# timdestan/go-raytracer

Measured on AMD Instinct MI355X. Metric: Mrays/s (primary+shadow+reflect) at 4K depth=6; 1/2/4/8-GPU scaling, higher is better.
Workload: dtype f64; 1 GPU; c3: cylinder + cube + sphere (cone substitute) over a reflective plane, 4 lights, 3840x2160, depth 6; width=3840, height=2160, depth=6, lights=4, objects=4, parallelism=rows1-interleaved, frames_in_flight=2, schedule=auto, kernel=specialised, accel=bvh+cull

## Files before the change

### go-raytracer_amd/csrc/rt_kernel.hip

```cpp
#pragma clang fp contract(off)

#include <hip/hip_runtime.h>

#include <dlfcn.h>
#include <errno.h>
#include <fcntl.h>
#include <hip/hiprtc.h>
#include <sys/syscall.h>
#include <sys/wait.h>
#include <unistd.h>

#include <algorithm>
#include <atomic>
#include <chrono>
#include <condition_variable>
#include <cstdlib>
#include <functional>
#include <thread>
#include <cmath>
#include <array>
#include <cstdio>
#include <utility>
#include <cstring>
#include <limits>
// ... 398 lines not shown

int align16(int v) { return (v + 15) & ~15; }

}

struct SpecKey {
  int lds = 1, bvh = 0, csg = 0, nobj = 0;
  std::string kinds;
  int kmask = 0, feat = 0, nlights = 0;
  int pow_bits = 7;
  int nocull = 0;
  int quads = 0;
  int share = 0;
  int far = 1;
  std::string str() const {
    return std::to_string(lds) + ":" + std::to_string(bvh) + ":" + std::to_string(csg) + ":" + std::to_string(nobj) + ":" + kinds + ":" +
           std::to_string(kmask) + ":" + std::to_string(feat) + ":" + std::to_string(nlights) + ":" + std::to_string(pow_bits) +
           ":" + std::to_string(nocull) + ":" + std::to_string(quads) + ":" + std::to_string(share) + ":" + std::to_string(far);
  }
};

struct LaunchPlan {
  const void* fn = nullptr;
  int shmem_fixed = -1, frames = 0, per_cu = 0, lds_levels = 0, lds_full = 0;
};

struct rt_context {
  int device = 0;
  int last_waves = 0, launches = 0;
  int sched = RT_SCHED_AUTO;
  int inflight = 1;
  LaunchPlan plan;
  unsigned long long* wdiag = nullptr;
  int cus = 0;
  int lds_per_cu = 0, lds_per_block = 0;
  int grid_lds = 0, grid_glb = 0;
  DevScene sc;
  bool has_scene = false;
  uint64_t* jump = nullptr;
  unsigned int* queue = nullptr;
  int qset = 0;
  unsigned long long* stats = nullptr;
  unsigned long long* stats_part = nullptr;
  int stats_parts = 0;
  double* stack = nullptr;
  double* vm_global = nullptr;
  size_t vm_global_bytes = 0;
// ... 1583 lines not shown
  const bool use_stream = !lds && !s.use_bvh && !s.has_csg && (spec_extra || !(spec && !(c->accel & RT_ACCEL_CULL)));
  const bool quads = sch == SCH_QUADS || (sch == SCH_PAIRS && !spec);
  const void* kfn = k_kernels[kernel_index(lds, s.use_bvh, s.has_csg, quads, s.ext_code)];
  const bool share = spec && share_m == RT_SHARE_GROUP;
  const int stream_off = board_off + (share ? BOARD_BYTES : 0);
  const int frames_off = stream_off + (use_stream ? WAVES_PER_WG * SCH * (GEO * (int)sizeof(double) + (int)sizeof(int)) : 0);
  int shmem = frames_off;
  auto occupancy = [&](int bytes) {
    int n = 0;
    if (spec) {
      if (hipModuleOccupancyMaxActiveBlocksPerMultiprocessor(&n, spec, WG, bytes) != hipSuccess) n = 0;
    } else if (hipOccupancyMaxActiveBlocksPerMultiprocessor(&n, kfn, WG, bytes) != hipSuccess) {
      n = 0;
    }
    return n;
  };
  const void* plan_fn = spec ? (const void*)spec : kfn;
  const int frames = std::max(1, s.depth - 1);
  LaunchPlan& pl = c->plan;
  const bool plan_hit = pl.fn == plan_fn && pl.shmem_fixed == shmem && pl.frames == frames;
  int per_cu = plan_hit ? pl.per_cu : occupancy(shmem);
  if (per_cu <= 0) per_cu = 1;
  const int level_bytes = WAVES_PER_WG * CORE * 64 * (int)sizeof(double);
  const int ext_bytes = WAVES_PER_WG * EXT_ROWS * 64 * (int)sizeof(double);
  int lds_levels = plan_hit ? pl.lds_levels : 0, lds_full = plan_hit ? pl.lds_full : 0;
  if (!plan_hit && c->lds_per_cu > 0 && c->lds_per_block > 0) {
    const int avail = std::min(c->lds_per_block, c->lds_per_cu / std::min(per_cu, 8)) - shmem;
    if (const char* e = rt_getenv("RT_LDS_FULL")) lds_full = std::max(0, std::min(frames, atoi(e)));
    while (lds_full > 0 && lds_full * (ext_bytes + level_bytes) > avail) lds_full--;
    lds_levels = std::max(lds_full, std::min(frames, (avail - lds_full * ext_bytes) / level_bytes));
    if (const char* e = rt_getenv("RT_LDS_LEVELS")) lds_levels = std::max(lds_full, std::min(lds_levels, atoi(e)));
    while (lds_levels > 0 && occupancy(shmem + lds_levels * level_bytes + lds_full * ext_bytes) < per_cu) {
      lds_levels--;
      lds_full = std::min(lds_full, lds_levels);
    }
  }
  if (!plan_hit) pl = LaunchPlan{plan_fn, shmem, frames, per_cu, lds_levels, lds_full};
  const int ext_off = shmem + lds_levels * level_bytes;
  shmem = ext_off + lds_full * ext_bytes;
  static const bool dbg = rt_getenv("RT_DEBUG_LAUNCH") != nullptr;
  if (dbg)
    fprintf(stderr, "[launch] blocks/CU %d, LDS/block %d B (fixed %d, frame cores %d levels, full frames %d levels), frames %d\n",
            per_cu, shmem, frames_off, lds_levels, lds_full, frames);
  const int grid = c->cus * std::min(per_cu, 8);
  c->last_waves = grid * WAVES_PER_WG;
  c->launches++;
  if (grid * WAVES_PER_WG > c->stack_waves) return fail(RT_E_INVALID, "frame stack smaller than the grid");
  if (spec && share_m == RT_SHARE_DEVICE) {
    const size_t need = (size_t)c->stack_waves * 64 * frames;
    if (need != c->gslots || frames != c->gframes) {
      (void)hipFree(c->gboard);
      c->gboard = nullptr;
      c->gslots = 0;
      if (hipExtMallocWithFlags((void**)&c->gboard, need * GS_REC * sizeof(uint64_t), hipDeviceMallocUncached) !=
          hipSuccess)
        return fail(RT_E_NOMEM, "device-wide work-sharing slots");
      if (!c->gring && hipExtMallocWithFlags((void**)&c->gring, (size_t)GS_RING * sizeof(uint64_t),
                                             hipDeviceMallocUncached) != hipSuccess)
        return fail(RT_E_NOMEM, "device-wide work-sharing ring");
      if (!c->gctl && hipExtMallocWithFlags((void**)&c->gctl, GS_CTL_U64 * sizeof(uint64_t), hipDeviceMallocUncached) !=
                          hipSuccess)
        return fail(RT_E_NOMEM, "device-wide work-sharing control");
      HIP_TRY(hipMemsetAsync(c->gboard, 0, need * GS_REC * sizeof(uint64_t), st));
      HIP_TRY(hipMemsetAsync(c->gring, 0, (size_t)GS_RING * sizeof(uint64_t), st));
      HIP_TRY(hipMemsetAsync(c->gctl, 0, GS_CTL_U64 * sizeof(uint64_t), st));
      c->gslots = need;
      c->gframes = frames;
    }
  }
  Params P;
  std::memset(&P, 0, sizeof P);
  P.lds_frames_off = frames_off;
  P.lds_levels = lds_levels;
  P.lds_full = lds_full;
  P.stream_off = stream_off;
  P.lds_ext_off = ext_off;
  P.qmask_off = qmask_off;
  P.jump_off = jump_off;
  P.board_off = board_off;
  P.gboard = c->gboard;
  P.gring = c->gring;
  P.gctl = c->gctl;
  P.gslots = c->gslots;
  P.gset = c->qset;
  P.off_geo = s.off_geo;
  P.off_shade = s.off_shade;
  P.off_mats = s.off_mats;
  P.off_lights = s.off_lights;
  P.off_kind = s.off_kind;
  P.off_objmat = s.off_objmat;
  P.off_pref = s.off_prefb;
  P.off_csg = s.off_csg;
  P.off_code = s.off_code;
  P.off_consts = s.off_consts;
  P.off_entry = s.off_entry;
  P.lds_vm_off = vm_off;
  P.vm_global = c->vm_global;
  P.blob_bytes = s.blob_bytes;
  P.jump = c->jump;
// ... 346 lines not shown
```

### go-raytracer_amd/csrc/rt_render.h

```cpp
#pragma once
#pragma clang fp contract(off)

#ifndef __HIPCC_RTC__
#include <hip/hip_runtime.h>
#endif

#include "rt_abi.h"
#include "rt_device.h"

#ifndef RT_CULL
#define RT_CULL 1
#endif
#ifndef RT_SHARE
#define RT_SHARE 0
#endif
#ifndef RT_PAIRS
#define RT_PAIRS 0
#endif
#ifndef RT_FAR_SHIFT
#define RT_FAR_SHIFT 1
#endif
#ifndef RT_GS_POLL
#define RT_GS_POLL 3
#endif
// ... 48 lines not shown
enum { SCH = 32 };
enum { SHADOW_CHECK = 8 };
enum { ST_SHADOW = 0, ST_TRACED = 1, ST_SHADED = 2, ST_SURFERR = 3, ST_STESTS = 4, ST_COUNT = ST_STESTS + RT_NUM_KINDS,
       ST_PHASE = 16, N_PHASE = 10, ST_BVHDIAG = 26, ST_EXDIAG = 34, ST_SHDIAG = 48, ST_PASSDIAG = 54,
       ST_CLOCKSTEP = 60, ST_LANEDIAG = 61 ,
       ST_WATCHDOG = 63,
       STATS_PART = 16  };
enum { SH_POST_S = 0, SH_POST_T = 1, SH_CLAIM = 2, SH_RECLAIM = 3, SH_WAIT = 4, SH_SPIN = 5 };
#ifdef RT_PHASE_TIMING
#define SHDIAG(k) atomicAdd(P.stats + ST_SHDIAG + (k), 1ull)
#else
#define SHDIAG(k) (void)0
#endif
enum { S_IDLE = 0, S_TRACE = 1, S_SHADE = 2, S_DONE = 3 };
enum { LDS_MAX_BYTES = 40 * 1024 };
enum { JUMP_ENTRIES = 20 * 4 };

__device__ __forceinline__ int est_x(int pts, unsigned int k) { return pts == 1 ? TILE / 2 : 2 + 4 * (int)(k & 1u); }
__device__ __forceinline__ int est_y(int pts, unsigned int k) { return pts == 1 ? TILE / 2 : 2 + 4 * (int)((k >> 1) & 1u); }

struct Params {
  int lds_frames_off;
  int lds_levels;
  int lds_full;
  int lds_ext_off;
  int stream_off;
  int qmask_off;
  int jump_off;
  int off_geo, off_shade, off_mats, off_lights, off_kind, off_objmat, off_pref, off_csg, off_code, off_consts,
      off_entry, blob_bytes;
  int lds_vm_off;
  double* vm_global;
  const uint64_t* jump;
  unsigned int* queue;
  unsigned int* queue_next;
  unsigned long long* stats;
  unsigned long long* stats_part;
  unsigned long long* wdiag;
  double* stack;
  uint32_t* out;
  int width, height, depth, nobj, nlights, y0, y1, tiles_x;
  int trow0, trow_stride;
  unsigned int total_slots;
  int frames;
  const float* bvh_nodes;
  const double* bvh_geo;
  const int* planes;
  int nplanes, bvh_stack_off;
// ... 34 lines not shown
            m[8] * d.x + m[9] * d.y + m[10] * d.z);
}
template <typename MP>
__device__ __forceinline__ Ray to_obj(MP m, const Ray& r) {
  Ray l;
  l.o = to_obj_o(m, r.o);
  l.d = to_obj_d(m, r.d);
  return l;
}
__device__ __forceinline__ bool ax_mag(double x, bool zero_ok) {
  const uint32_t e = ((uint32_t)__double2hiint(x) >> 20) & 0x7ffu;
  return e - 123u < 1800u || (zero_ok && x == 0.0);
}
__device__ __forceinline__ bool axis_o_ok(d3 o) { return ax_mag(o.x, true) && ax_mag(o.y, true) && ax_mag(o.z, true); }
__device__ __forceinline__ bool axis_d_ok(d3 d) { return ax_mag(d.x, false) && ax_mag(d.y, false) && ax_mag(d.z, false); }
__device__ __forceinline__ d3 axis_o(const double* a, d3 o) {
  return mk(a[0] * o.x + a[1], a[2] * o.y + a[3], a[4] * o.z + a[5]);
}
__device__ __forceinline__ d3 axis_d(const double* a, d3 d) { return mk(a[0] * d.x, a[2] * d.y, a[4] * d.z); }

typedef const __attribute__((address_space(4))) double* cdptr;
typedef const __attribute__((address_space(4))) float* cfptr;
typedef const __attribute__((address_space(4))) int* ciptr;
__device__ __forceinline__ const float* as_f(const double* p) { return reinterpret_cast<const float*>(p); }
__device__ __forceinline__ cfptr as_f(cdptr p) { return (cfptr)p; }
__device__ __forceinline__ const int* as_i(const double* p) { return reinterpret_cast<const int*>(p); }
__device__ __forceinline__ ciptr as_i(cdptr p) { return (ciptr)p; }
template <int N>
struct RecN {
  double m[N];
};
typedef RecN<12> Rec12;
typedef RecN<6> Rec6;
typedef RecN<3> Rec3;
enum { AXIS_REC = 8, UNI_REC = 4 };
template <int N, typename PT>
__device__ __forceinline__ RecN<N> ld_rec(PT p) {
  RecN<N> r;
#pragma unroll
  for (int q = 0; q < N; q++) r.m[q] = p[q];
  return r;
}
struct LeafRec {
  RecN<12> R;
  float cx, cy, cz, cr;
  int i, k;
// ... 820 lines not shown
    uint64_t t_ = stamp();                \
    asm volatile("; @phase_end " #k ::: "memory"); \
    ph_acc[k] += t_ - ph_t0_;             \
    ph_t0_ = t_;                          \
  } while (0)
#else
#define PH_BEGIN() (void)0
#define PH_MARK(k) (void)0
#endif

#ifdef RT_EXACT_DIAG
#define EXDIAG(k, sh, b)                                                                    \
  do {                                                                                      \
    const uint64_t act_ = wave_ballot(1), m_ = wave_ballot(b);                                    \
    if ((int)(threadIdx.x & 63) == __ffsll((long long)act_) - 1) {                          \
      atomicAdd(P.stats + ST_EXDIAG + 2 * (k) + (sh), (unsigned long long)__popcll(m_));    \
      atomicAdd(P.stats + ST_EXDIAG + 2 * RT_NUM_KINDS + (sh), 1ull);                       \
    }                                                                                       \
  } while (0)
#else
#define EXDIAG(k, sh, b) (void)0
#endif

__device__ __forceinline__ double* frame_ptr(double* base, int frame) { return base + (size_t)frame * FRAME_FIELDS * 64; }
__device__ __forceinline__ void st3(double* f, int field, d3 v) {
  f[(field + 0) * 64] = v.x;
  f[(field + 1) * 64] = v.y;
  f[(field + 2) * 64] = v.z;
}
__device__ __forceinline__ d3 ld3(const double* f, int field) {
  return mk(f[(field + 0) * 64], f[(field + 1) * 64], f[(field + 2) * 64]);
}

__device__ __forceinline__ int core_gfield(int c) { return c < 3 ? c : (c == 3 ? 9 : 10); }

enum { FL_TMODE = 1, FL_HASR = 2, FL_HAST = 4, FL_STAGE = 8, FL_VMMAT = 16, FL_FORKED = 32, FL_TASK = 64 };
enum { PK_SLOT = 8, PK_MAT = 32 };
#define PK_SLOT_OF(packed) ((int)(((packed) >> PK_SLOT) & 0xffffff))

enum { SHARE_SPINS = 1 << 16,
       SHARE_SLEEP = 127,
       SHARE_SAMPLES = 1 };
enum { NSLOT = 64, SLOTS_PER_WAVE = NSLOT / WAVES_PER_WG, S_WAIT = 4, S_RESUME = 5 };
enum { S_ADV = 6 };
struct Board {
  unsigned long long post;
  unsigned long long done;
  unsigned int wfree[WAVES_PER_WG];
  int nidle;
  int nactive;
  int pad[2];
  double ray[NSLOT][6];
  int meta[NSLOT][2];
  uint32_t lw[WG];
};
__device__ __forceinline__ int lw_own_end(uint32_t w) { return (int)(w & 7u); }
__device__ __forceinline__ int lw_task(uint32_t w) { return (int)((w >> 3) & 127u) - 1; }
// ... 286 lines not shown
  S.mats = reinterpret_cast<const double*>(base + P.off_mats);
  const double* G = reinterpret_cast<const double*>(base + P.off_lights);
  S.lights = G + GLOB;
  S.kind = reinterpret_cast<const int*>(base + P.off_kind);
  S.objmat = reinterpret_cast<const int*>(base + P.off_objmat);
  S.pref = reinterpret_cast<const uint32_t*>(base + P.off_pref);
  S.csg = reinterpret_cast<const int*>(base + P.off_csg);
  S.code = reinterpret_cast<const uint32_t*>(base + P.off_code);
  S.entry = reinterpret_cast<const int*>(base + P.off_entry);
  S.consts = reinterpret_cast<const uint64_t*>(base + P.off_consts);
#ifdef RT_SPEC_NOBJ
  const cdptr sgeo = (cdptr)(blob + P.off_geo);
#endif
  const cdptr cs_geo = (cdptr)(blob + P.off_geo);
  const ciptr cs_kind = (ciptr)(blob + P.off_kind);
  const ciptr cs_csg = (ciptr)(blob + P.off_csg);
#define CSG_ARGS cs_geo, cs_kind, cs_csg
#define CSG_G(i, g) (cs_geo + (size_t)(i) * GEO)
#define LTP(li) (S.lights + (size_t)(li) * LGT)
#define SHP(i) (S.shade + (size_t)(i) * SHD)

  const int lane = (int)(threadIdx.x & 63);
  const int wslot = (int)(blockIdx.x * WAVES_PER_WG + (threadIdx.x >> 6));
  double* stk = P.stack + (size_t)wslot * ((size_t)P.frames * FRAME_FIELDS * 64) + lane;
  const int lds_lv = P.lds_levels;
  double* lfr = reinterpret_cast<double*>(smem + P.lds_frames_off) +
                (size_t)(threadIdx.x >> 6) * (lds_lv * CORE * 64) + lane;
  auto core_ld = [&](int level, int c) -> double {
    if (level < lds_lv) return lfr[(level * CORE + c) * 64];
    return frame_ptr(stk, level)[core_gfield(c) * 64];
  };
  const int lds_full = P.lds_full;
  double* lext = reinterpret_cast<double*>(smem + P.lds_ext_off) + (size_t)(threadIdx.x >> 6) * (lds_full * EXT_ROWS * 64) + lane;
  auto ext = [&](int level) -> double* {
    return level < lds_full ? lext + (size_t)level * EXT_ROWS * 64 : frame_ptr(stk, level) + FR_EXT * 64;
  };
  auto core_st = [&](int level, int c, double v) {
    if (level < lds_lv)
      lfr[(level * CORE + c) * 64] = v;
    else
      frame_ptr(stk, level)[core_gfield(c) * 64] = v;
  };
  double* vmrec;
  if constexpr (LDS)
    vmrec = reinterpret_cast<double*>(smem + P.lds_vm_off) + (size_t)threadIdx.x * MAT;
  else
    vmrec = P.vm_global + ((size_t)wslot * 64 + lane) * MAT;
  constexpr bool STREAM = !LDS && !BVH && !CSG;
  double* sbuf = reinterpret_cast<double*>(smem + P.stream_off) + (size_t)(threadIdx.x >> 6) * (SCH * GEO);
  int* skind = reinterpret_cast<int*>(smem + P.stream_off + WAVES_PER_WG * SCH * GEO * (int)sizeof(double)) +
               (threadIdx.x >> 6) * SCH;
  auto stream_objects = [&](auto&& body) {
    constexpr int PER = SCH * GEO * (int)sizeof(double) / 16 / 64;
    const uint4* src = reinterpret_cast<const uint4*>(S.geo);
    uint4* dst = reinterpret_cast<uint4*>(sbuf);
    const int lane_ = (int)(threadIdx.x & 63);
    uint4 pre[PER];
    int pk = 0;
    auto fetch = [&](int c0) {
      const int n16 = min(SCH, P.nobj - c0) * (GEO * (int)sizeof(double) / 16);
#pragma unroll
      for (int q = 0; q < PER; q++) {
        const int idx = lane_ + q * 64;
        pre[q] = idx < n16 ? src[(size_t)c0 * (GEO * sizeof(double) / 16) + idx] : make_uint4(0, 0, 0, 0);
// ... 89 lines not shown
  uint32_t lane_cost = 0;
#endif
#endif

  const double W1 = (double)(P.width - 1), H1 = (double)(P.height - 1);

  auto gen_ray = [&]() {
    double dx = pcg_float64(rng) - 0.5;
    double dy = pcg_float64(rng) - 0.5;
    const double vw = G[9], vh = G[10];
    double u = ((double)px + dx) / W1 * vw - vw / 2.0;
    double v = ((double)py + dy) / H1 * vh - vh / 2.0;
    ray.o = mk(u, -v, 0.0);
    ray.d = norm(sub(ray.o, eye));
  };

  auto sample_rng = [&](int x, int y, int k) {
    const int ry = y % 20;
    const uint64_t* j = P.jump + (ry * 4 + k) * 4;
    return pcg_jump(Pcg{0xDEADULL ^ (uint64_t)x, 0xBEEFULL ^ (uint64_t)(y - ry)}, j[0], j[1], j[2], j[3]);
  };
  auto wait_slot = [&]() -> int {
    if (RT_SHARE == 1 && !QD && sp == 0) return lw_fork(Bd->lw[threadIdx.x], sample);
    return PK_SLOT_OF(__double_as_longlong(core_ld(sp - 1, 4)));
  };
  auto advance_sample = [&](uint32_t w) {
    for (;;) {
      if (P.est_out && sample == 1) {
        state = S_IDLE;
        return;
      }
      if (PR && sample == ((lane & 1) ? 4 : 2)) {
        state = S_DONE;
        return;
      }
      if (sample == 4) {
        d3 c = scale(sum, 1.0 / 4.0);
        uint32_t r8 = go_f64_to_u32(c.x * 65535.0) >> 8;
        uint32_t g8 = go_f64_to_u32(c.y * 65535.0) >> 8;
        uint32_t b8 = go_f64_to_u32(c.z * 65535.0) >> 8;
#ifdef RT_COST_MAP
        P.out[pout] = lane_cost;
        lane_cost = 0;
#else
        const uint32_t v = (r8 & 0xffu) | ((g8 & 0xffu) << 8) | ((b8 & 0xffu) << 16) | 0xff000000u;
        held_px = pout;
        held_val = v;
// ... 23 lines not shown
      }
      sum = add(sum, board_take(Bd, q));
      sample++;
    }
  };

  auto unwind = [&](bool have_res, d3 res, bool pf_valid, long long pf_packed, d3 pf_lw, double pf_kr) {
    while (wave_any(have_res)) {
      if (have_res) {
        if (sp == 0) {
          if constexpr (QD) {
            sum = res;
            state = S_DONE;
          } else {
            if (PR && (lane & 1))
              (sample == 2 ? sum : sum2) = res;
            else
              sum = add(sum, res);
            sample++;
            state = S_ADV;
          }
          have_res = false;
        } else {
          double* f = frame_ptr(stk, sp - 1);
          long long packed;
          if (pf_valid)
            packed = pf_packed;
          else
            packed = __double_as_longlong(core_ld(sp - 1, 4));
          int fl = (int)(packed & 0xff);
          if (RT_SHARE && __builtin_expect((fl & FL_TASK) != 0, 0)) {
            if constexpr (RT_SHARE == 2)
              gs_deliver(P.gboard, PK_SLOT_OF(packed), res);
            else
              board_deliver(Bd, PK_SLOT_OF(packed), res);
            sp = 0;
            state = S_IDLE;
            have_res = false;
          } else if ((fl & FL_HASR) && (fl & FL_HAST) && !(fl & FL_STAGE)) {
            double* e = ext(sp - 1);
            const d3 first = res;
            bool here = true;
            core_st(sp - 1, 4, __longlong_as_double(packed | FL_STAGE));
            if (RT_SHARE && __builtin_expect((fl & FL_FORKED) != 0, 0)) {
              const int q = PK_SLOT_OF(packed);
              if (RT_SHARE == 2 ? gs_reclaim(P.gboard, q) : board_reclaim(Bd, q)) {
                SHDIAG(SH_RECLAIM);
                if (RT_SHARE == 1) board_free(Bd, q);
              } else if (RT_SHARE == 2 ? gs_done(P.gboard, q) : board_done(Bd, q)) {
                here = false;
                res = RT_SHARE == 2 ? gs_take(P.gboard, q) : board_take(Bd, q);
              } else {
                SHDIAG(SH_WAIT);
                here = false;
                state = S_WAIT;
                have_res = false;
              }
            }
            if (here) {
              ray.o = ld3(e, 0);
              ray.d = ld3(e, 3);
              state = S_TRACE;
              have_res = false;
            }
            st3(e, 0, first);
          } else {
            const double* FM = S.mats + (size_t)(packed >> PK_MAT) * MAT;
            d3 R = mk(0, 0, 0), Tr = mk(0, 0, 0);
            if ((fl & FL_HASR) && (fl & FL_HAST)) {
              R = ld3(ext(sp - 1), 0);
              Tr = res;
            } else if (fl & FL_HASR) {
              R = res;
            } else {
              Tr = res;
            }
            d3 lw;
            double kr;
            if (pf_valid) {
              lw = pf_lw;
              kr = pf_kr;
            } else {
              lw = mk(core_ld(sp - 1, 0), core_ld(sp - 1, 1), core_ld(sp - 1, 2));
              kr = core_ld(sp - 1, 3);
            }
            d3 fcol;
            double frefl;
            if (spec_feat(SF_VM) && (fl & FL_VMMAT)) {
              fcol = ld3(f, FR_COL);
              frefl = f[FR_REFL * 64];
            } else {
              fcol = mk(FM[0], FM[1], FM[2]);
              frefl = FM[3];
            }
            res = combine((fl & FL_TMODE) != 0, lw, fcol, frefl, kr, R, Tr);
            sp--;
          }
          pf_valid = false;
        }
      }
    }
  };

  PH_BEGIN();
#ifdef RT_PHASE_TIMING
  const uint64_t life_t0 = ph_t0_;
  uint64_t last_grab = life_t0, nchunk_taken = 0;
#endif
  uint32_t guard_iters = 0;
  for (;;) {
    if (++guard_iters > (1u << 26)) {
      if (lane == 0) atomicAdd(P.stats + ST_WATCHDOG, 1ull);
      break;
// ... 170 lines not shown
        if (lane == 0) {
          gt = gs_ld(g_tail);
          if (!gs_helper || (guard_iters & 7u) == 0u || gt != gs_t) {
            nid = (int)gs_ld32(g_nidle);
            gh = gs_ld(g_head);
          } else {
            nid = gs_nid;
            gh = gs_h;
          }
        }
        gs_nid = __builtin_amdgcn_readfirstlane(nid);
        gs_h = rfl64(gh);
        gs_t = rfl64(gt);
      }
      const int nid = gs_nid;
      const uint64_t gh = gs_h, gt = gs_t;
      const long long outstanding = (long long)(gt - gh);
      const int want = nid - (int)min(outstanding, (long long)(1 << 30));
      if (__builtin_expect(want > 0 && outstanding < GS_RSH / 2, 0)) {
        const bool busy_lane = state == S_TRACE || state == S_SHADE || state == S_WAIT;
        int L = -1;
        if (busy_lane)
          for (int l = min(sp - 1, P.depth - 1 - GS_MIN_LEVELS); l >= 0; l--) {
            const int f = (int)(__double_as_longlong(core_ld(l, 4)) & 0xff);
            if (f & FL_TASK) break;
            if ((f & (FL_HASR | FL_HAST | FL_STAGE | FL_FORKED)) == (FL_HASR | FL_HAST)) L = l;
          }
        const uint64_t cm = wave_ballot(L >= 0);
        if (cm) {
          const int npost = min((int)__popcll(cm), want);
          const int rk = (int)__builtin_amdgcn_mbcnt_hi((unsigned int)(cm >> 32),
                                                        __builtin_amdgcn_mbcnt_lo((unsigned int)cm, 0u));
          const bool post = L >= 0 && rk < npost;
          int q = 0;
          if (post) {
            SHDIAG(SH_POST_T);
            q = (wslot * 64 + lane) * P.frames + L;
            uint64_t* r = gs_slot(P.gboard, q);
            const double* e = ext(L);
            const d3 o = ld3(e, 0), dd = ld3(e, 3);
            gs_st(r + 0, (uint64_t)__double_as_longlong(o.x));
            gs_st(r + 1, (uint64_t)__double_as_longlong(o.y));
            gs_st(r + 2, (uint64_t)__double_as_longlong(o.z));
            gs_st(r + 3, (uint64_t)__double_as_longlong(dd.x));
            gs_st(r + 4, (uint64_t)__double_as_longlong(dd.y));
            gs_st(r + 5, (uint64_t)__double_as_longlong(dd.z));
            gs_st(r + 6, (uint64_t)(L + 1));
            gs_drain();
            gs_st(r + 7, GS_POSTED);
            const long long pk = __double_as_longlong(core_ld(L, 4));
            core_st(L, 4, __longlong_as_double(pk | FL_FORKED | ((long long)q << PK_SLOT)));
          }
          gs_drain();
          uint64_t t0 = 0;
          if (lane == 0) t0 = __hip_atomic_fetch_add(g_tail, (uint64_t)npost, __ATOMIC_RELAXED, RT_AG_SCOPE);
          t0 = rfl64(t0);
          if (post) {
            const uint64_t t = t0 + (uint64_t)rk;
            gs_st(g_ring + (t & (GS_RSH - 1)), (t << 32) | (uint32_t)q);
          }
        }
      }
      uint64_t il = exhausted ? wave_ballot(state == S_IDLE) : 0ull;
      int cshard = gshard;
      uint64_t ch = gh;
      bool ctry = outstanding > 0;
      if (GS_SH > 1 && il != 0 && !ctry && gs_helper && (guard_iters & 3u) == 0u && !P.est_out) {
        const int k = lane < GS_SH ? (gshard + 1 + lane) % GS_SH : gshard;
        uint64_t ot = 0, oh = 0;
        if (lane < GS_SH - 1) {
          ot = gs_ld(P.gctl + GS_SHARD * k + GS_TAIL);
          oh = gs_ld(P.gctl + GS_SHARD * k + GS_HEAD);
        }
        const uint64_t hasm = wave_ballot(lane < GS_SH - 1 && ot > oh);
// ... 28 lines not shown
        h = rfl64(h);
        k = __builtin_amdgcn_readfirstlane(k);
        if (k > 0) {
          const int rk = (int)__builtin_amdgcn_mbcnt_hi((unsigned int)(il >> 32),
                                                        __builtin_amdgcn_mbcnt_lo((unsigned int)il, 0u));
          if (state == S_IDLE && rk < k) {
            const uint64_t t = h + (uint64_t)rk;
            uint64_t e = 0;
            for (int w_ = 0; w_ < (1 << 14); w_++) {
              e = gs_ld(c_ring + (t & (GS_RSH - 1)));
              if ((uint32_t)(e >> 32) == (uint32_t)t) break;
              __builtin_amdgcn_s_sleep(1);
            }
            if ((uint32_t)(e >> 32) == (uint32_t)t && (uint32_t)e < P.gslots) {
              const int q = (int)(uint32_t)e;
              uint64_t* r = gs_slot(P.gboard, q);
              if (gs_claim(r)) {
                SHDIAG(SH_CLAIM);
                ray.o = mk(__longlong_as_double((long long)gs_ld(r + 0)), __longlong_as_double((long long)gs_ld(r + 1)),
                           __longlong_as_double((long long)gs_ld(r + 2)));
                ray.d = mk(__longlong_as_double((long long)gs_ld(r + 3)), __longlong_as_double((long long)gs_ld(r + 4)),
                           __longlong_as_double((long long)gs_ld(r + 5)));
                const int m0 = (int)gs_ld(r + 6);
                core_st(m0 - 1, 4, __longlong_as_double((long long)FL_TASK | ((long long)q << PK_SLOT)));
                sp = m0;
                state = S_TRACE;
              }
            }
          }
          il = wave_ballot(state == S_IDLE);
        }
      }
      const int cur_idle = (exhausted && !P.est_out) ? (int)__popcll(il) : 0;
      if (cur_idle != my_idle) {
        nidle_add(cur_idle - my_idle);
        my_idle = cur_idle;
      }
      const bool busy = wave_any(state != S_IDLE);
      if (busy != my_active) {
        if (lane == 0) atomicAdd(g_active, busy ? 1u : 0xffffffffu);
        my_active = busy;
      }
      if (__builtin_expect(!busy, 0)) {
        if (!gs_helper) {
          unsigned int old = 0;
          if (lane == 0) old = atomicAdd(g_helpers, 1u);
          gs_helper = __builtin_amdgcn_readfirstlane((int)old) < RT_GS_HELPERS;
// ... 13 lines not shown
        __builtin_amdgcn_s_sleep(SHARE_SLEEP);
        continue;
      }
      spins = 0;
      if (__builtin_expect(!wave_any(state == S_TRACE || state == S_SHADE || state == S_RESUME), 0)) {
        __builtin_amdgcn_s_sleep(SHARE_SLEEP / 4);
        continue;
      }
    } else if constexpr (RT_SHARE == 1) {
      if (__builtin_expect(wave_any(state == S_WAIT), 0)) {
        if (state == S_WAIT && board_done(Bd, wait_slot())) state = S_RESUME;
      }
      const int nid = __builtin_amdgcn_readfirstlane(__hip_atomic_load(&Bd->nidle, __ATOMIC_RELAXED, RT_WG_SCOPE));
      const uint64_t pmp = nid > 0 ? __hip_atomic_load(&Bd->post, __ATOMIC_RELAXED, RT_WG_SCOPE) : 0ull;
      const int want = nid - (int)__popcll(((uint64_t)__builtin_amdgcn_readfirstlane((int)(pmp >> 32)) << 32) |
                                           (uint32_t)__builtin_amdgcn_readfirstlane((int)pmp));
      if (__builtin_expect(want > 0, 0)) {
        const bool busy_lane = state == S_TRACE || state == S_SHADE || state == S_WAIT;
        const uint32_t w = busy_lane ? Bd->lw[threadIdx.x] : 0u;
        const bool cs = !QD && SHARE_SAMPLES && busy_lane && lw_task(w) < 0 && lw_own_end(w) - 1 > sample;
        int L = -1;
        if (busy_lane && !cs)
          for (int l = sp - 1; l >= 0; l--) {
            const int f = (int)(__double_as_longlong(core_ld(l, 4)) & 0xff);
            if (f & FL_TASK) break;
            if ((f & (FL_HASR | FL_HAST | FL_STAGE | FL_FORKED)) == (FL_HASR | FL_HAST)) L = l;
          }
        const bool cand = cs || L >= 0;
        const uint64_t cm = wave_ballot(cand);
        if (cm) {
          const uint32_t wf = (uint32_t)__builtin_amdgcn_readfirstlane(
              (int)__hip_atomic_load(&Bd->wfree[wave], __ATOMIC_RELAXED, RT_WG_SCOPE));
          const int npost = min(min((int)__popcll(cm), (int)__popc(wf)), want);
          if (npost > 0) {
            const uint32_t used = (uint32_t)low_bits(wf, npost);
            const int rk = (int)__builtin_amdgcn_mbcnt_hi((unsigned int)(cm >> 32),
                                                          __builtin_amdgcn_mbcnt_lo((unsigned int)cm, 0u));
            if (cand && rk < npost) {
              const int q = wave * SLOTS_PER_WAVE + nth_bit(wf, rk);
              if (cs) {
                SHDIAG(SH_POST_S);
                const int k = lw_own_end(w) - 1;
                Bd->meta[q][0] = px | (k << 16) | META_SAMPLE;
                Bd->meta[q][1] = py;
                const int sh = 10 + 6 * (k - 1);
                Bd->lw[threadIdx.x] = (w & ~7u & ~(63u << sh)) | (uint32_t)k | ((uint32_t)q << sh);
              } else {
                SHDIAG(SH_POST_T);
                const double* e = ext(L);
                const d3 o = ld3(e, 0), dd = ld3(e, 3);
                Bd->ray[q][0] = o.x;
                Bd->ray[q][1] = o.y;
                Bd->ray[q][2] = o.z;
                Bd->ray[q][3] = dd.x;
                Bd->ray[q][4] = dd.y;
                Bd->ray[q][5] = dd.z;
                Bd->meta[q][0] = L + 1;
                Bd->meta[q][1] = 0;
                const long long pk = __double_as_longlong(core_ld(L, 4));
                core_st(L, 4, __longlong_as_double(pk | FL_FORKED | ((long long)q << PK_SLOT)));
              }
            }
            if (lane == 0) {
              __hip_atomic_fetch_and(&Bd->wfree[wave], ~used, __ATOMIC_RELAXED, RT_WG_SCOPE);
              __hip_atomic_fetch_or(&Bd->post, (uint64_t)used << (wave * SLOTS_PER_WAVE), __ATOMIC_RELEASE,
                                    RT_WG_SCOPE);
            }
          }
        }
      }
      uint64_t il = exhausted ? wave_ballot(state == S_IDLE) : 0ull;
      if (__builtin_expect(il != 0, 0)) {
        const uint64_t pm0 = __hip_atomic_load(&Bd->post, __ATOMIC_RELAXED, RT_WG_SCOPE);
        const uint64_t pm = ((uint64_t)__builtin_amdgcn_readfirstlane((int)(pm0 >> 32)) << 32) |
                            (uint32_t)__builtin_amdgcn_readfirstlane((int)pm0);
        if (pm) {
          const uint64_t want = low_bits(pm, (int)__popcll(il));
          uint64_t old = 0;
          if (lane == 0) old = __hip_atomic_fetch_and(&Bd->post, ~want, __ATOMIC_ACQUIRE, RT_WG_SCOPE);
          const uint64_t got = want & (((uint64_t)__builtin_amdgcn_readfirstlane((int)(old >> 32)) << 32) |
                                       (uint32_t)__builtin_amdgcn_readfirstlane((int)old));
          const int rk = (int)__builtin_amdgcn_mbcnt_hi((unsigned int)(il >> 32),
                                                        __builtin_amdgcn_mbcnt_lo((unsigned int)il, 0u));
          if (state == S_IDLE && rk < (int)__popcll(got)) {
            const int q = nth_bit(got, rk);
            SHDIAG(SH_CLAIM);
            const int m0 = Bd->meta[q][0];
            if (m0 & META_SAMPLE) {
              px = m0 & 0xffff;
              py = Bd->meta[q][1];
              sample = (m0 >> 16) & 3;
              Bd->lw[threadIdx.x] = (uint32_t)(sample + 1) | ((uint32_t)(q + 1) << 3);
              sum = mk(-0.0, -0.0, -0.0);
              rng = sample_rng(px, py, sample);
              need_gen = true;
              sp = 0;
            } else {
              ray.o = mk(Bd->ray[q][0], Bd->ray[q][1], Bd->ray[q][2]);
              ray.d = mk(Bd->ray[q][3], Bd->ray[q][4], Bd->ray[q][5]);
              core_st(m0 - 1, 4, __longlong_as_double((long long)FL_TASK | ((long long)q << PK_SLOT)));
              Bd->lw[threadIdx.x] = 0u;
              sp = m0;
            }
            state = S_TRACE;
          }
          il = wave_ballot(state == S_IDLE);
        }
      }
      const int cur_idle = P.est_out ? 0 : (int)__popcll(il);
      if (cur_idle != my_idle) {
        if (lane == 0) __hip_atomic_fetch_add(&Bd->nidle, cur_idle - my_idle, __ATOMIC_RELAXED, RT_WG_SCOPE);
        my_idle = cur_idle;
      }
      const bool busy = wave_any(state != S_IDLE);
      if (busy != my_active) {
        if (lane == 0) __hip_atomic_fetch_add(&Bd->nactive, busy ? 1 : -1, __ATOMIC_RELAXED, RT_WG_SCOPE);
        my_active = busy;
      }
      if (__builtin_expect(!busy, 0)) {
        const int na = __builtin_amdgcn_readfirstlane(__hip_atomic_load(&Bd->nactive, __ATOMIC_RELAXED, RT_WG_SCOPE));
        const uint64_t pm = __hip_atomic_load(&Bd->post, __ATOMIC_RELAXED, RT_WG_SCOPE);
        if ((na == 0 && __builtin_amdgcn_readfirstlane((int)(pm >> 32)) == 0 &&
             __builtin_amdgcn_readfirstlane((int)pm) == 0) ||
// ... 20 lines not shown
    ld_rounds++;
#endif
    PH_MARK(0);
    if (wave_any(need_gen)) {
#ifdef RT_PHASE_TIMING
      pd_gen++;
      pd_genl += (uint64_t)__popcll(wave_ballot(need_gen));
#endif
      if (need_gen) {
        gen_ray();
        need_gen = false;
      }
    }
    PH_MARK(1);

    if (wave_any(state == S_TRACE || (RT_SHARE && state == S_RESUME))) {
      const bool tr = state == S_TRACE;
      bool pf = false;
      long long pf_packed = 0;
      d3 pf_lw = mk(0, 0, 0);
      double pf_kr = 0.0;
      if (tr && sp > 0) {
        pf = true;
        pf_packed = __double_as_longlong(core_ld(sp - 1, 4));
        pf_lw = mk(core_ld(sp - 1, 0), core_ld(sp - 1, 1), core_ld(sp - 1, 2));
        pf_kr = core_ld(sp - 1, 3);
      }
      bool found = false;
      double best_t = 0.0;
      int best_i = 0, best_f = 0;
      const F3 of = f3(ray.o), df = f3(ray.d);
      const float slack = ray_slack(of);
      auto trace_exact = [&](int i, int k, const double* g, bool test) {
        EXDIAG(k, 0, test);
        if (test) {
          double t;
          int f;
          bool h;
          if constexpr (CSG)
            h = k == RT_CSG ? csg_hit<EXT>(CSG_ARGS, P.nobj, CSG_G(i, g), ray, t, f, 1.0,
                                      found ? best_t : __builtin_inf(), true)
                            : object_hit(k, g, ray, t, f);
          else
            h = object_hit(k, g, ray, t, f);
          if (h) {
            if (!found || t < best_t || (BVH && t == best_t && i < best_i)) {
              found = true;
              best_t = t;
              best_i = i;
// ... 700 lines not shown
          if (dot(ray.d, nn) > 0.0) {
            ratio = M[8];
            nn = scale(nn, -1.0);
          }
          double cosI = -dot(nn, ray.d);
          double sinT2 = ratio * ratio * (1.0 - cosI * cosI);
          if (!(sinT2 > 1.0)) {
            double cosT = gsqrt(1.0 - sinT2);
            d3 td = add(scale(ray.d, ratio), scale(nn, ratio * cosI - cosT));
            if (!iszero(td)) {
              hasT = true;
              trr.o = sub(pw, scale(nn, 1e-4));
              trr.d = td;
            }
          }
          double cosi = dot(ray.d, nw) / (rlen * len(nw));
          const double r0 = M[13];
          double cost = __builtin_fabs(cosi);
          kr = r0 + (1 - r0) * go_pow(1 - cost, 5);
          lw = scale(L, 1.0 - T);
        }
        const int d = P.depth - sp;
        if (d - 1 > 0 && (hasR || hasT)) {
          core_st(sp, 0, lw.x);
          core_st(sp, 1, lw.y);
          core_st(sp, 2, lw.z);
          if (hasR && hasT) {
            st3(ext(sp), 0, trr.o);
            st3(ext(sp), 3, trr.d);
          }
          core_st(sp, 3, kr);
          if (spec_feat(SF_VM) && mat < 0) {
            double* f = frame_ptr(stk, sp);
            st3(f, FR_COL, col);
            f[FR_REFL * 64] = refl;
          }
          long long packed = ((long long)(mat < 0 ? 0 : mat) << PK_MAT) | (mat < 0 ? FL_VMMAT : 0) |
                             (tmode ? FL_TMODE : 0) | (hasR ? FL_HASR : 0) | (hasT ? FL_HAST : 0);
          core_st(sp, 4, __longlong_as_double(packed));
          sp++;
          ray = hasR ? rr : trr;
          state = S_TRACE;
        } else {
          res = combine(tmode, lw, col, refl, kr, mk(0, 0, 0), mk(0, 0, 0));
          have_res = true;
        }
      }
    }
    PH_MARK(8);
    unwind(have_res, res, false, 0, mk(0, 0, 0), 0.0);
    PH_MARK(9);
  }
  flush_pixels();

  if (lane == 0) {
#ifdef RT_PHASE_TIMING
    for (int k = 0; k < N_PHASE; k++) atomicAdd(P.stats + ST_PHASE + k, (unsigned long long)ph_acc[k]);
    atomicAdd(P.stats + ST_BVHDIAG + 0, (unsigned long long)bd_tnodes);
    atomicAdd(P.stats + ST_BVHDIAG + 1, (unsigned long long)bd_snodes);
    atomicAdd(P.stats + ST_BVHDIAG + 2, (unsigned long long)bd_tleaf);
    atomicAdd(P.stats + ST_BVHDIAG + 3, (unsigned long long)bd_sleaf);
    atomicAdd(P.stats + ST_BVHDIAG + 4, (unsigned long long)bd_trays);
// ... 42 lines not shown
```

Measured before the change: 73080 Mrays/s.

## Drop LDS ext-frame tier and address frame stack with explicit global/LDS pointers

Removes the LDS tier for the extended frame rows (second-ray origin and direction), so they always live in the global per-lane frame stack. The LDS budget goes entirely to core levels. Frame and core accesses now use typed address-space pointers with a mid-frame byte offset and umul24 indexing, so the compiler can emit direct global/LDS instructions with small immediate offsets. Core load and store are grouped into single helpers, and the unwind path reuses the prefetched values. This cuts address arithmetic and generic-pointer overhead, but the ext rows now always go to global memory.

```diff
diff --git a/go-raytracer_amd/csrc/rt_kernel.hip b/go-raytracer_amd/csrc/rt_kernel.hip
--- a/go-raytracer_amd/csrc/rt_kernel.hip
+++ b/go-raytracer_amd/csrc/rt_kernel.hip
@@ -444,7 +444,7 @@
 
 struct LaunchPlan {
   const void* fn = nullptr;
-  int shmem_fixed = -1, frames = 0, per_cu = 0, lds_levels = 0, lds_full = 0;
+  int shmem_fixed = -1, frames = 0, per_cu = 0, lds_levels = 0;
 };
 
 struct rt_context {
@@ -2074,26 +2074,19 @@
   int per_cu = plan_hit ? pl.per_cu : occupancy(shmem);
   if (per_cu <= 0) per_cu = 1;
   const int level_bytes = WAVES_PER_WG * CORE * 64 * (int)sizeof(double);
-  const int ext_bytes = WAVES_PER_WG * EXT_ROWS * 64 * (int)sizeof(double);
-  int lds_levels = plan_hit ? pl.lds_levels : 0, lds_full = plan_hit ? pl.lds_full : 0;
+  int lds_levels = plan_hit ? pl.lds_levels : 0;
   if (!plan_hit && c->lds_per_cu > 0 && c->lds_per_block > 0) {
     const int avail = std::min(c->lds_per_block, c->lds_per_cu / std::min(per_cu, 8)) - shmem;
-    if (const char* e = rt_getenv("RT_LDS_FULL")) lds_full = std::max(0, std::min(frames, atoi(e)));
-    while (lds_full > 0 && lds_full * (ext_bytes + level_bytes) > avail) lds_full--;
-    lds_levels = std::max(lds_full, std::min(frames, (avail - lds_full * ext_bytes) / level_bytes));
-    if (const char* e = rt_getenv("RT_LDS_LEVELS")) lds_levels = std::max(lds_full, std::min(lds_levels, atoi(e)));
-    while (lds_levels > 0 && occupancy(shmem + lds_levels * level_bytes + lds_full * ext_bytes) < per_cu) {
-      lds_levels--;
-      lds_full = std::min(lds_full, lds_levels);
-    }
-  }
-  if (!plan_hit) pl = LaunchPlan{plan_fn, shmem, frames, per_cu, lds_levels, lds_full};
-  const int ext_off = shmem + lds_levels * level_bytes;
-  shmem = ext_off + lds_full * ext_bytes;
+    lds_levels = std::max(0, std::min(frames, avail / level_bytes));
+    if (const char* e = rt_getenv("RT_LDS_LEVELS")) lds_levels = std::max(0, std::min(lds_levels, atoi(e)));
+    while (lds_levels > 0 && occupancy(shmem + lds_levels * level_bytes) < per_cu) lds_levels--;
+  }
+  if (!plan_hit) pl = LaunchPlan{plan_fn, shmem, frames, per_cu, lds_levels};
+  shmem += lds_levels * level_bytes;
   static const bool dbg = rt_getenv("RT_DEBUG_LAUNCH") != nullptr;
   if (dbg)
-    fprintf(stderr, "[launch] blocks/CU %d, LDS/block %d B (fixed %d, frame cores %d levels, full frames %d levels), frames %d\n",
-            per_cu, shmem, frames_off, lds_levels, lds_full, frames);
+    fprintf(stderr, "[launch] blocks/CU %d, LDS/block %d B (fixed %d, frame cores %d levels), frames %d\n", per_cu, shmem,
+            frames_off, lds_levels, frames);
   const int grid = c->cus * std::min(per_cu, 8);
   c->last_waves = grid * WAVES_PER_WG;
   c->launches++;
@@ -2124,9 +2117,7 @@
   std::memset(&P, 0, sizeof P);
   P.lds_frames_off = frames_off;
   P.lds_levels = lds_levels;
-  P.lds_full = lds_full;
   P.stream_off = stream_off;
-  P.lds_ext_off = ext_off;
   P.qmask_off = qmask_off;
   P.jump_off = jump_off;
   P.board_off = board_off;
diff --git a/go-raytracer_amd/csrc/rt_render.h b/go-raytracer_amd/csrc/rt_render.h
--- a/go-raytracer_amd/csrc/rt_render.h
+++ b/go-raytracer_amd/csrc/rt_render.h
@@ -94,8 +94,6 @@
 struct Params {
   int lds_frames_off;
   int lds_levels;
-  int lds_full;
-  int lds_ext_off;
   int stream_off;
   int qmask_off;
   int jump_off;
@@ -176,6 +174,8 @@
 typedef const __attribute__((address_space(4))) double* cdptr;
 typedef const __attribute__((address_space(4))) float* cfptr;
 typedef const __attribute__((address_space(4))) int* ciptr;
+typedef __attribute__((address_space(3))) double* ldptr;
+typedef __attribute__((address_space(1))) double* gdptr;
 __device__ __forceinline__ const float* as_f(const double* p) { return reinterpret_cast<const float*>(p); }
 __device__ __forceinline__ cfptr as_f(cdptr p) { return (cfptr)p; }
 __device__ __forceinline__ const int* as_i(const double* p) { return reinterpret_cast<const int*>(p); }
@@ -1042,17 +1042,21 @@
 #define EXDIAG(k, sh, b) (void)0
 #endif
 
-__device__ __forceinline__ double* frame_ptr(double* base, int frame) { return base + (size_t)frame * FRAME_FIELDS * 64; }
-__device__ __forceinline__ void st3(double* f, int field, d3 v) {
-  f[(field + 0) * 64] = v.x;
-  f[(field + 1) * 64] = v.y;
-  f[(field + 2) * 64] = v.z;
-}
-__device__ __forceinline__ d3 ld3(const double* f, int field) {
-  return mk(f[(field + 0) * 64], f[(field + 1) * 64], f[(field + 2) * 64]);
-}
-
-__device__ __forceinline__ int core_gfield(int c) { return c < 3 ? c : (c == 3 ? 9 : 10); }
+enum { FRAME_MID = FRAME_FIELDS / 2, FRAME_BYTES = FRAME_FIELDS * 64 * 8 };
+__device__ __forceinline__ gdptr frame_ptr(gdptr base, uint32_t lane8, int frame) {
+  typedef __attribute__((address_space(1))) char* gbptr;
+  return (gdptr)((gbptr)base + (__umul24((uint32_t)frame, (uint32_t)FRAME_BYTES) + lane8));
+}
+__device__ __forceinline__ __attribute__((address_space(1))) double& fr(gdptr f, int field) { return f[(field - FRAME_MID) * 64]; }
+__device__ __forceinline__ void st3(gdptr f, int field, d3 v) {
+  fr(f, field + 0) = v.x;
+  fr(f, field + 1) = v.y;
+  fr(f, field + 2) = v.z;
+}
+__device__ __forceinline__ d3 ld3(gdptr f, int field) { return mk(fr(f, field + 0), fr(f, field + 1), fr(f, field + 2)); }
+
+__device__ __forceinline__ constexpr int core_gfield(int c) { return c < 3 ? c : (c == 3 ? 9 : 10); }
+enum { CF_LW = 0, CF_KR = 3, CF_PACKED = 4 };
 
 enum { FL_TMODE = 1, FL_HASR = 2, FL_HAST = 4, FL_STAGE = 8, FL_VMMAT = 16, FL_FORKED = 32, FL_TASK = 64 };
 enum { PK_SLOT = 8, PK_MAT = 32 };
@@ -1385,24 +1389,51 @@
 
   const int lane = (int)(threadIdx.x & 63);
   const int wslot = (int)(blockIdx.x * WAVES_PER_WG + (threadIdx.x >> 6));
-  double* stk = P.stack + (size_t)wslot * ((size_t)P.frames * FRAME_FIELDS * 64) + lane;
+  const gdptr stk = (gdptr)P.stack + (size_t)__builtin_amdgcn_readfirstlane(wslot) * ((size_t)P.frames * FRAME_FIELDS * 64);
+  uint32_t lane8 = (uint32_t)lane * 8u + FRAME_MID * 512u;
+  asm volatile("" : "+v"(lane8));
+  auto frame = [&](int level) -> gdptr { return frame_ptr(stk, lane8, level); };
   const int lds_lv = P.lds_levels;
-  double* lfr = reinterpret_cast<double*>(smem + P.lds_frames_off) +
-                (size_t)(threadIdx.x >> 6) * (lds_lv * CORE * 64) + lane;
-  auto core_ld = [&](int level, int c) -> double {
-    if (level < lds_lv) return lfr[(level * CORE + c) * 64];
-    return frame_ptr(stk, level)[core_gfield(c) * 64];
+  typedef __attribute__((address_space(3))) char* lbptr;
+  const lbptr lfr = (lbptr)(smem + P.lds_frames_off) + ((int)(threadIdx.x >> 6) * (lds_lv * CORE * 512) + lane * 8);
+  auto lcore = [&](int level) -> ldptr { return (ldptr)(lfr + __umul24((uint32_t)level, (uint32_t)(CORE * 512))); };
+  auto core_load = [&](int level, long long& packed, d3& lw, double& kr) {
+    if (level < lds_lv) {
+      const ldptr p = lcore(level);
+      lw = mk(p[(CF_LW + 0) * 64], p[(CF_LW + 1) * 64], p[(CF_LW + 2) * 64]);
+      kr = p[CF_KR * 64];
+      packed = __double_as_longlong(p[CF_PACKED * 64]);
+    } else {
+      const gdptr f = frame(level);
+      lw = ld3(f, core_gfield(CF_LW));
+      kr = fr(f, core_gfield(CF_KR));
+      packed = __double_as_longlong(fr(f, core_gfield(CF_PACKED)));
+    }
   };
-  const int lds_full = P.lds_full;
-  double* lext = reinterpret_cast<double*>(smem + P.lds_ext_off) + (size_t)(threadIdx.x >> 6) * (lds_full * EXT_ROWS * 64) + lane;
-  auto ext = [&](int level) -> double* {
-    return level < lds_full ? lext + (size_t)level * EXT_ROWS * 64 : frame_ptr(stk, level) + FR_EXT * 64;
+  auto core_store = [&](int level, long long packed, d3 lw, double kr) {
+    if (level < lds_lv) {
+      const ldptr p = lcore(level);
+      p[(CF_LW + 0) * 64] = lw.x;
+      p[(CF_LW + 1) * 64] = lw.y;
+      p[(CF_LW + 2) * 64] = lw.z;
+      p[CF_KR * 64] = kr;
+      p[CF_PACKED * 64] = __longlong_as_double(packed);
+    } else {
+      const gdptr f = frame(level);
+      st3(f, core_gfield(CF_LW), lw);
+      fr(f, core_gfield(CF_KR)) = kr;
+      fr(f, core_gfield(CF_PACKED)) = __longlong_as_double(packed);
+    }
   };
-  auto core_st = [&](int level, int c, double v) {
+  auto packed_ld = [&](int level) -> long long {
+    if (level < lds_lv) return __double_as_longlong(lcore(level)[CF_PACKED * 64]);
+    return __double_as_longlong(fr(frame(level), core_gfield(CF_PACKED)));
+  };
+  auto packed_st = [&](int level, long long packed) {
     if (level < lds_lv)
-      lfr[(level * CORE + c) * 64] = v;
+      lcore(level)[CF_PACKED * 64] = __longlong_as_double(packed);
     else
-      frame_ptr(stk, level)[core_gfield(c) * 64] = v;
+      fr(frame(level), core_gfield(CF_PACKED)) = __longlong_as_double(packed);
   };
   double* vmrec;
   if constexpr (LDS)
@@ -1538,7 +1569,7 @@
   };
   auto wait_slot = [&]() -> int {
     if (RT_SHARE == 1 && !QD && sp == 0) return lw_fork(Bd->lw[threadIdx.x], sample);
-    return PK_SLOT_OF(__double_as_longlong(core_ld(sp - 1, 4)));
+    return PK_SLOT_OF(packed_ld(sp - 1));
   };
   auto advance_sample = [&](uint32_t w) {
     for (;;) {
@@ -1608,12 +1639,9 @@
           }
           have_res = false;
         } else {
-          double* f = frame_ptr(stk, sp - 1);
-          long long packed;
-          if (pf_valid)
-            packed = pf_packed;
-          else
-            packed = __double_as_longlong(core_ld(sp - 1, 4));
+          const gdptr f = frame(sp - 1);
+          if (!pf_valid) core_load(sp - 1, pf_packed, pf_lw, pf_kr);
+          const long long packed = pf_packed;
           int fl = (int)(packed & 0xff);
           if (RT_SHARE && __builtin_expect((fl & FL_TASK) != 0, 0)) {
             if constexpr (RT_SHARE == 2)
@@ -1624,10 +1652,9 @@
             state = S_IDLE;
             have_res = false;
           } else if ((fl & FL_HASR) && (fl & FL_HAST) && !(fl & FL_STAGE)) {
-            double* e = ext(sp - 1);
             const d3 first = res;
             bool here = true;
-            core_st(sp - 1, 4, __longlong_as_double(packed | FL_STAGE));
+            packed_st(sp - 1, packed | FL_STAGE);
             if (RT_SHARE && __builtin_expect((fl & FL_FORKED) != 0, 0)) {
               const int q = PK_SLOT_OF(packed);
               if (RT_SHARE == 2 ? gs_reclaim(P.gboard, q) : board_reclaim(Bd, q)) {
@@ -1644,37 +1671,30 @@
               }
             }
             if (here) {
-              ray.o = ld3(e, 0);
-              ray.d = ld3(e, 3);
+              ray.o = ld3(f, FR_EXT);
+              ray.d = ld3(f, FR_EXT + 3);
               state = S_TRACE;
               have_res = false;
             }
-            st3(e, 0, first);
+            st3(f, FR_EXT, first);
           } else {
             const double* FM = S.mats + (size_t)(packed >> PK_MAT) * MAT;
             d3 R = mk(0, 0, 0), Tr = mk(0, 0, 0);
             if ((fl & FL_HASR) && (fl & FL_HAST)) {
-              R = ld3(ext(sp - 1), 0);
+              R = ld3(f, FR_EXT);
               Tr = res;
             } else if (fl & FL_HASR) {
               R = res;
             } else {
               Tr = res;
             }
-            d3 lw;
-            double kr;
-            if (pf_valid) {
-              lw = pf_lw;
-              kr = pf_kr;
-            } else {
-              lw = mk(core_ld(sp - 1, 0), core_ld(sp - 1, 1), core_ld(sp - 1, 2));
-              kr = core_ld(sp - 1, 3);
-            }
+            const d3 lw = pf_lw;
+            const double kr = pf_kr;
             d3 fcol;
             double frefl;
             if (spec_feat(SF_VM) && (fl & FL_VMMAT)) {
               fcol = ld3(f, FR_COL);
-              frefl = f[FR_REFL * 64];
+              frefl = fr(f, FR_REFL);
             } else {
               fcol = mk(FM[0], FM[1], FM[2]);
               frefl = FM[3];
@@ -1891,7 +1911,7 @@
         int L = -1;
         if (busy_lane)
           for (int l = min(sp - 1, P.depth - 1 - GS_MIN_LEVELS); l >= 0; l--) {
-            const int f = (int)(__double_as_longlong(core_ld(l, 4)) & 0xff);
+            const int f = (int)(packed_ld(l) & 0xff);
             if (f & FL_TASK) break;
             if ((f & (FL_HASR | FL_HAST | FL_STAGE | FL_FORKED)) == (FL_HASR | FL_HAST)) L = l;
           }
@@ -1906,8 +1926,8 @@
             SHDIAG(SH_POST_T);
             q = (wslot * 64 + lane) * P.frames + L;
             uint64_t* r = gs_slot(P.gboard, q);
-            const double* e = ext(L);
-            const d3 o = ld3(e, 0), dd = ld3(e, 3);
+            const gdptr e = frame(L);
+            const d3 o = ld3(e, FR_EXT), dd = ld3(e, FR_EXT + 3);
             gs_st(r + 0, (uint64_t)__double_as_longlong(o.x));
             gs_st(r + 1, (uint64_t)__double_as_longlong(o.y));
             gs_st(r + 2, (uint64_t)__double_as_longlong(o.z));
@@ -1917,8 +1937,8 @@
             gs_st(r + 6, (uint64_t)(L + 1));
             gs_drain();
             gs_st(r + 7, GS_POSTED);
-            const long long pk = __double_as_longlong(core_ld(L, 4));
-            core_st(L, 4, __longlong_as_double(pk | FL_FORKED | ((long long)q << PK_SLOT)));
+            const long long pk = packed_ld(L);
+            packed_st(L, pk | FL_FORKED | ((long long)q << PK_SLOT));
           }
           gs_drain();
           uint64_t t0 = 0;
@@ -1993,7 +2013,7 @@
                 ray.d = mk(__longlong_as_double((long long)gs_ld(r + 3)), __longlong_as_double((long long)gs_ld(r + 4)),
                            __longlong_as_double((long long)gs_ld(r + 5)));
                 const int m0 = (int)gs_ld(r + 6);
-                core_st(m0 - 1, 4, __longlong_as_double((long long)FL_TASK | ((long long)q << PK_SLOT)));
+                packed_st(m0 - 1, (long long)FL_TASK | ((long long)q << PK_SLOT));
                 sp = m0;
                 state = S_TRACE;
               }
@@ -2053,7 +2073,7 @@
         int L = -1;
         if (busy_lane && !cs)
           for (int l = sp - 1; l >= 0; l--) {
-            const int f = (int)(__double_as_longlong(core_ld(l, 4)) & 0xff);
+            const int f = (int)(packed_ld(l) & 0xff);
             if (f & FL_TASK) break;
             if ((f & (FL_HASR | FL_HAST | FL_STAGE | FL_FORKED)) == (FL_HASR | FL_HAST)) L = l;
           }
@@ -2078,8 +2098,8 @@
                 Bd->lw[threadIdx.x] = (w & ~7u & ~(63u << sh)) | (uint32_t)k | ((uint32_t)q << sh);
               } else {
                 SHDIAG(SH_POST_T);
-                const double* e = ext(L);
-                const d3 o = ld3(e, 0), dd = ld3(e, 3);
+                const gdptr e = frame(L);
+                const d3 o = ld3(e, FR_EXT), dd = ld3(e, FR_EXT + 3);
                 Bd->ray[q][0] = o.x;
                 Bd->ray[q][1] = o.y;
                 Bd->ray[q][2] = o.z;
@@ -2088,8 +2108,8 @@
                 Bd->ray[q][5] = dd.z;
                 Bd->meta[q][0] = L + 1;
                 Bd->meta[q][1] = 0;
-                const long long pk = __double_as_longlong(core_ld(L, 4));
-                core_st(L, 4, __longlong_as_double(pk | FL_FORKED | ((long long)q << PK_SLOT)));
+                const long long pk = packed_ld(L);
+                packed_st(L, pk | FL_FORKED | ((long long)q << PK_SLOT));
               }
             }
             if (lane == 0) {
@@ -2129,7 +2149,7 @@
             } else {
               ray.o = mk(Bd->ray[q][0], Bd->ray[q][1], Bd->ray[q][2]);
               ray.d = mk(Bd->ray[q][3], Bd->ray[q][4], Bd->ray[q][5]);
-              core_st(m0 - 1, 4, __longlong_as_double((long long)FL_TASK | ((long long)q << PK_SLOT)));
+              packed_st(m0 - 1, (long long)FL_TASK | ((long long)q << PK_SLOT));
               Bd->lw[threadIdx.x] = 0u;
               sp = m0;
             }
@@ -2196,9 +2216,7 @@
       double pf_kr = 0.0;
       if (tr && sp > 0) {
         pf = true;
-        pf_packed = __double_as_longlong(core_ld(sp - 1, 4));
-        pf_lw = mk(core_ld(sp - 1, 0), core_ld(sp - 1, 1), core_ld(sp - 1, 2));
-        pf_kr = core_ld(sp - 1, 3);
+        core_load(sp - 1, pf_packed, pf_lw, pf_kr);
       }
       bool found = false;
       double best_t = 0.0;
@@ -2945,22 +2963,19 @@
         }
         const int d = P.depth - sp;
         if (d - 1 > 0 && (hasR || hasT)) {
-          core_st(sp, 0, lw.x);
-          core_st(sp, 1, lw.y);
-          core_st(sp, 2, lw.z);
           if (hasR && hasT) {
-            st3(ext(sp), 0, trr.o);
-            st3(ext(sp), 3, trr.d);
-          }
-          core_st(sp, 3, kr);
+            const gdptr f = frame(sp);
+            st3(f, FR_EXT, trr.o);
+            st3(f, FR_EXT + 3, trr.d);
+          }
           if (spec_feat(SF_VM) && mat < 0) {
-            double* f = frame_ptr(stk, sp);
+            const gdptr f = frame(sp);
             st3(f, FR_COL, col);
-            f[FR_REFL * 64] = refl;
+            fr(f, FR_REFL) = refl;
           }
           long long packed = ((long long)(mat < 0 ? 0 : mat) << PK_MAT) | (mat < 0 ? FL_VMMAT : 0) |
                              (tmode ? FL_TMODE : 0) | (hasR ? FL_HASR : 0) | (hasT ? FL_HAST : 0);
-          core_st(sp, 4, __longlong_as_double(packed));
+          core_store(sp, packed, lw, kr);
           sp++;
           ray = hasR ? rr : trr;
           state = S_TRACE;
```

New measurement: 74930 Mrays/s (median of 6 runs). 2.5% higher.
